# Anttwo/SuGaR

Hardware: NVIDIA B200
Metric: forward+backward views/sec @3M Gaussians 1920x1080 (higher is better)
Workload: dtype f32

## Files before the change

### sugar_b200/csrc/sgr_backward.cu

```cuda
#include <mutex>

#include "sgr_internal.cuh"

namespace sgr {

#ifndef SGR_BWD_PIPE3
#define SGR_BWD_PIPE3 1
#endif
#ifndef SGR_BWD_NS
#define SGR_BWD_NS 3
#endif
#ifndef SGR_BWD_B
#define SGR_BWD_B (SGR_BWD_PIPE3 ? 96 : 128)
#endif
constexpr int BWD_B = SGR_BWD_B;
constexpr int BWD_NW = 8;

__device__ __forceinline__ void red_add_v4(float *addr, float a, float b, float c, float d)
{
    asm volatile("red.global.add.v4.f32 [%0], {%1, %2, %3, %4};" ::"l"(addr), "f"(a), "f"(b), "f"(c), "f"(d) : "memory");
}
__device__ __forceinline__ void red_add_v2(float *addr, float a, float b)
{
    asm volatile("red.global.add.v2.f32 [%0], {%1, %2};" ::"l"(addr), "f"(a), "f"(b) : "memory");
// ... 304 lines not shown
                        dL_dalpha = fmaf(Cc.x - acc1, dp.y, dL_dalpha);
                        dL_dalpha = fmaf(Cc.y - acc2, dp.z, dL_dalpha);
                        dL_dalpha *= T;
                        dL_dalpha = fmaf(dp.w, inv, dL_dalpha);
                        S = B.z * dL_dalpha * G;
                        acc0 = fmaf(alpha, B.w, om * acc0);
                        acc1 = fmaf(alpha, Cc.x, om * acc1);
                        acc2 = fmaf(alpha, Cc.y, om * acc2);
                    }
                }
                sts64(cb + (lane * CH_PITCH + nfill) * 8, S, dchannel);
                const uint32_t ma = cb + CB_META + nfill * 32;
                sts128(ma, A.x, A.y, A.z, A.w);
                {
                    const float2 Cm = lds64(sc + j * 16 + 8);
                    sts128(ma + 16, B.x, B.z, Cm.x, Cm.y);
                }
                if (++nfill == CH) {
                    chunk_flush(cb, CH, blk_x0, blk_y0, 0.5f * W, 0.5f * H, gacc, dcol);
                    nfill = 0;
                }
            }
        }
#if SGR_BWD_PIPE3
        __syncwarp();
        if (lane == 0) mbar_arrive(&bars[NS + buf]);
#endif
    }
    if (nfill) chunk_flush(cb, nfill, blk_x0, blk_y0, 0.5f * W, 0.5f * H, gacc, dcol);
}

struct PreBwdArgs {
    int p0, p1;
    const float *means, *scales, *rots, *shs, *cov_pre;
    ViewConsts v;
    const int32_t *radii;
    const float *gacc;
    const float *dcol;
    float *dmeans2D, *dopacity, *dmeans3D, *dcov3D, *dsh, *dscales, *drots;
    float *rec11;
    int in_bulk_ok, out_bulk_ok, sh_stride, sh_vec;
    const float *sh_rest;
    const float4 *rec;
    float *dsh_rest;
    const float *const *view_tab;
    int nviews, my_view;
    size_t campos_off;
    float dsh_scale;
    float *const *stage_tab;
    int pf_off;
};

#define SH_C0 0.28209479177387814f
#define SH_C1 0.4886025119029199f
__constant__ float b_SH_C2[5] = {1.0925484305920792f, -1.0925484305920792f, 0.31539156525252005f,
                                 -1.0925484305920792f, 0.5462742152960396f};
__constant__ float b_SH_C3[7] = {-0.5900435899266435f, 2.890611442640554f, -0.4570457994644658f,
                                 0.3731763325901154f, -0.4570457994644658f, 1.445305721320277f,
                                 -0.5900435899266435f};

struct f3 {
    float x, y, z;
};

template <bool OTHERS = false>
__device__ __forceinline__ void sh_backward_inplace(int deg, int M, float *dc, float *rest, f3 dir_orig, f3 dRGB,
                                                    f3 &dmean, float out_scale = 1.0f, const float *oacc = nullptr)
{
    const f3 dS = {dRGB.x * out_scale, dRGB.y * out_scale, dRGB.z * out_scale};
    const float len = sqrtf(dir_orig.x * dir_orig.x + dir_orig.y * dir_orig.y + dir_orig.z * dir_orig.z);
    const float x = dir_orig.x / len, y = dir_orig.y / len, z = dir_orig.z / len;
    float ddx = 0.f, ddy = 0.f, ddz = 0.f;
#define SHB(k, w, cx, cy, cz)                                                          \
    {                                                                                  \
        float *q_ = (k) == 0 ? dc : rest + ((k) - 1) * 3;                              \
        const float t_ = q_[0] * dRGB.x + q_[1] * dRGB.y + q_[2] * dRGB.z;             \
        ddx += (cx) * t_;                                                              \
        ddy += (cy) * t_;                                                              \
        ddz += (cz) * t_;                                                              \
        const float w_ = (w);                                                          \
        if (OTHERS) {  \
            q_[0] = fmaf(w_, dS.x, oacc[(k) * 3]);                                     \
            q_[1] = fmaf(w_, dS.y, oacc[(k) * 3 + 1]);                                 \
            q_[2] = fmaf(w_, dS.z, oacc[(k) * 3 + 2]);                                 \
        } else {                                                                       \
            q_[0] = w_ * dS.x;                                                         \
            q_[1] = w_ * dS.y;                                                         \
            q_[2] = w_ * dS.z;                                                         \
        }                                                                              \
    }
    SHB(0, SH_C0, 0.f, 0.f, 0.f);
    if (deg > 0) {
        SHB(1, -SH_C1 * y, 0.f, -SH_C1, 0.f);
        SHB(2, SH_C1 * z, 0.f, 0.f, SH_C1);
        SHB(3, -SH_C1 * x, -SH_C1, 0.f, 0.f);
        if (deg > 1) {
            const float xx = x * x, yy = y * y, zz = z * z, xy = x * y, yz = y * z, xz = x * z;
            SHB(4, b_SH_C2[0] * xy, b_SH_C2[0] * y, b_SH_C2[0] * x, 0.f);
            SHB(5, b_SH_C2[1] * yz, 0.f, b_SH_C2[1] * z, b_SH_C2[1] * y);
            SHB(6, b_SH_C2[2] * (2.f * zz - xx - yy), b_SH_C2[2] * 2.f * -x, b_SH_C2[2] * 2.f * -y, b_SH_C2[2] * 2.f * 2.f * z);
            SHB(7, b_SH_C2[3] * xz, b_SH_C2[3] * z, 0.f, b_SH_C2[3] * x);
            SHB(8, b_SH_C2[4] * (xx - yy), b_SH_C2[4] * 2.f * x, b_SH_C2[4] * 2.f * -y, 0.f);
            if (deg > 2) {
                SHB(9, b_SH_C3[0] * y * (3.f * xx - yy), b_SH_C3[0] * 3.f * 2.f * xy, b_SH_C3[0] * 3.f * (xx - yy), 0.f);
                SHB(10, b_SH_C3[1] * xy * z, b_SH_C3[1] * yz, b_SH_C3[1] * xz, b_SH_C3[1] * xy);
                SHB(11, b_SH_C3[2] * y * (4.f * zz - xx - yy), b_SH_C3[2] * -2.f * xy,
                    b_SH_C3[2] * (-3.f * yy + 4.f * zz - xx), b_SH_C3[2] * 4.f * 2.f * yz);
                SHB(12, b_SH_C3[3] * z * (2.f * zz - 3.f * xx - 3.f * yy), b_SH_C3[3] * -3.f * 2.f * xz,
                    b_SH_C3[3] * -3.f * 2.f * yz, b_SH_C3[3] * 3.f * (2.f * zz - xx - yy));
                SHB(13, b_SH_C3[4] * x * (4.f * zz - xx - yy), b_SH_C3[4] * (-3.f * xx + 4.f * zz - yy),
                    b_SH_C3[4] * -2.f * xy, b_SH_C3[4] * 4.f * 2.f * xz);
                SHB(14, b_SH_C3[5] * z * (xx - yy), b_SH_C3[5] * 2.f * xz, b_SH_C3[5] * -2.f * yz, b_SH_C3[5] * (xx - yy));
                SHB(15, b_SH_C3[6] * x * (xx - 3.f * yy), b_SH_C3[6] * 3.f * (xx - yy), b_SH_C3[6] * -3.f * 2.f * xy, 0.f);
            }
        }
    }
#undef SHB
    for (int k = (deg + 1) * (deg + 1) * 3 - 3; k < (M - 1) * 3; k++) rest[k] = 0.f;
    const f3 o = dir_orig;
    const float sum2 = o.x * o.x + o.y * o.y + o.z * o.z;
    const float invsum32 = 1.0f / sqrtf(sum2 * sum2 * sum2);
    dmean.x += ((+sum2 - o.x * o.x) * ddx - o.y * o.x * ddy - o.z * o.x * ddz) * invsum32;
    dmean.y += (-o.x * o.y * ddx + (sum2 - o.y * o.y) * ddy - o.z * o.y * ddz) * invsum32;
    dmean.z += (-o.x * o.z * ddx - o.y * o.z * ddy + (sum2 - o.z * o.z) * ddz) * invsum32;
}

__device__ __forceinline__ void sh_accumulate(int deg, float *acc, f3 dir_orig, f3 g)
{
    const float inv = 1.0f / sqrtf(dir_orig.x * dir_orig.x + dir_orig.y * dir_orig.y + dir_orig.z * dir_orig.z);
    const float x = dir_orig.x * inv, y = dir_orig.y * inv, z = dir_orig.z * inv;
#define SHA(k, w)                                           \
    {                                                       \
        const float w_ = (w);                               \
        acc[(k) * 3] = fmaf(w_, g.x, acc[(k) * 3]);         \
        acc[(k) * 3 + 1] = fmaf(w_, g.y, acc[(k) * 3 + 1]); \
        acc[(k) * 3 + 2] = fmaf(w_, g.z, acc[(k) * 3 + 2]); \
    }
    SHA(0, SH_C0);
    if (deg > 0) {
        SHA(1, -SH_C1 * y);
        SHA(2, SH_C1 * z);
        SHA(3, -SH_C1 * x);
        if (deg > 1) {
            const float xx = x * x, yy = y * y, zz = z * z, xy = x * y, yz = y * z, xz = x * z;
            SHA(4, b_SH_C2[0] * xy);
            SHA(5, b_SH_C2[1] * yz);
            SHA(6, b_SH_C2[2] * (2.f * zz - xx - yy));
            SHA(7, b_SH_C2[3] * xz);
            SHA(8, b_SH_C2[4] * (xx - yy));
            if (deg > 2) {
                SHA(9, b_SH_C3[0] * y * (3.f * xx - yy));
// ... 35 lines not shown
__device__ __forceinline__ void bulk_s2g(void *dst, const void *src_smem, uint32_t bytes)
{
    asm volatile("cp.async.bulk.global.shared::cta.bulk_group [%0], [%1], %2;" ::"l"(dst), "r"(smem_u32(src_smem)),
                 "r"(bytes)
                 : "memory");
}

__device__ __forceinline__ void pb_stage(float *dst, const float *__restrict__ src, int n)
{
    for (int i = threadIdx.x; i < n; i += PB_T) dst[i] = __ldg(src + i);
}
__device__ __forceinline__ void pb_flush(float *__restrict__ dst, const float *src, int n)
{
    for (int i = threadIdx.x; i < n; i += PB_T) dst[i] = src[i];
}

template <bool RAW, bool MULTI = false>
__global__ void __launch_bounds__(PB_T) preprocess_backward_kernel(const PreBwdArgs a)
{
    extern __shared__ __align__(16) float sm[];
    __shared__ __align__(8) uint64_t s_bar;
    const int tid = threadIdx.x;
    const int base = a.p0 + blockIdx.x * PB_T;
    const int n = min(PB_T, a.p1 - base);
    const int i = base + tid;
    const int M = a.v.M;
    const bool full = (n == PB_T);

    if (a.in_bulk_ok && full) {
        if (tid == 0) {
            mbar_init(&s_bar, 1);
            mbar_fence_init();
            uint32_t bytes = PB_T * 32 + PB_T * 12;
            if (a.shs) bytes += PB_T * 12;
            if (RAW && a.shs) bytes += PB_T * 12 + PB_T * (uint32_t)(a.v.M - 1) * 12;
            if (a.scales) bytes += PB_T * 12 + PB_T * 16;
            if (a.cov_pre) bytes += PB_T * 24;
            const int pulled = MULTI ? min(a.nviews - 1, PB_VB) : 0;
            bytes += (uint32_t)pulled * PB_T * 12;
            mbar_expect_tx(&s_bar, bytes);
            for (int u = 0; u < pulled; u++) {
                const int v = u + (u >= a.my_view ? 1 : 0);
                bulk_g2s(sm + a.pf_off + u * PB_T * 3, a.view_tab[v] + (size_t)base * 3, PB_T * 12, &s_bar);
            }
            if (RAW && a.shs) {
                bulk_g2s(sm + PB_SHDC, a.shs + (size_t)base * 3, PB_T * 12, &s_bar);
                if (a.v.M > 1)
                    bulk_g2s(sm + PB_SH, a.sh_rest + (size_t)base * (a.v.M - 1) * 3, PB_T * (uint32_t)(a.v.M - 1) * 12, &s_bar);
            }
            bulk_g2s(sm + PB_GACC, a.gacc + (size_t)base * 8, PB_T * 32, &s_bar);
            if (a.shs) bulk_g2s(sm + PB_DCOL, a.dcol + (size_t)base * 3, PB_T * 12, &s_bar);
            bulk_g2s(sm + PB_MEANS, a.means + (size_t)base * 3, PB_T * 12, &s_bar);
            if (a.scales) {
                bulk_g2s(sm + PB_SCALES, a.scales + (size_t)base * 3, PB_T * 12, &s_bar);
                bulk_g2s(sm + PB_ROTS, a.rots + (size_t)base * 4, PB_T * 16, &s_bar);
            }
            if (a.cov_pre) bulk_g2s(sm + PB_COV, a.cov_pre + (size_t)base * 6, PB_T * 24, &s_bar);
        }
    } else {
        pb_stage(sm + PB_GACC, a.gacc + (size_t)base * 8, n * 8);
        if (a.shs) pb_stage(sm + PB_DCOL, a.dcol + (size_t)base * 3, n * 3);
        pb_stage(sm + PB_MEANS, a.means + (size_t)base * 3, n * 3);
        if (a.scales) {
            pb_stage(sm + PB_SCALES, a.scales + (size_t)base * 3, n * 3);
            pb_stage(sm + PB_ROTS, a.rots + (size_t)base * 4, n * 4);
        }
        if (a.cov_pre) pb_stage(sm + PB_COV, a.cov_pre + (size_t)base * 6, n * 6);
        if (RAW && a.shs) {
            pb_stage(sm + PB_SHDC, a.shs + (size_t)base * 3, n * 3);
            pb_stage(sm + PB_SH, a.sh_rest + (size_t)base * (M - 1) * 3, n * (M - 1) * 3);
        }
        if (MULTI) {
            const int pulled = min(a.nviews - 1, PB_VB);
            for (int u = 0; u < pulled; u++) {
                const int v = u + (u >= a.my_view ? 1 : 0);
                pb_stage(sm + a.pf_off + u * PB_T * 3, a.view_tab[v] + (size_t)base * 3, n * 3);
            }
        }
    }
    float *s_sh = sm + PB_SH;
    const int row_f = RAW ? (M - 1) * 3 : M * 3;
    if (!RAW && a.shs) {
        const float *src = a.shs + (size_t)base * row_f;
        if (a.sh_vec) {
            const int row_v = row_f >> 2, total = n * row_v;
            int r = tid / row_v, c = tid - r * row_v;
            const int dr = PB_T / row_v, dc = PB_T - dr * row_v;
            for (int k = tid; k < total; k += PB_T) {
                cp_async16(s_sh + r * a.sh_stride + c * 4, src + (size_t)k * 4);
                r += dr;
                c += dc;
                if (c >= row_v) {
                    c -= row_v;
                    r++;
                }
            }
        } else {
            const int total = n * row_f;
            for (int k = tid; k < total; k += PB_T) {
                const int r = k / row_f, c = k - r * row_f;
                cp_async4(s_sh + r * a.sh_stride + c, src + k);
            }
        }
        cp_async_commit();
    }
    int radius = 0;
    if (tid < n) radius = a.radii[i];
    const int others = MULTI ? a.nviews - 1 : 0;
    __syncthreads();
    if (a.in_bulk_ok && full) mbar_wait(&s_bar, 0);
    if (!RAW && a.shs) {
        cp_async_wait<0>();
        __syncthreads();
    }

    float oacc[MULTI ? 48 : 1];
    auto sum_other_views = [&]() {
        if (!MULTI) return;
#pragma unroll
        for (int k = 0; k < (MULTI ? 48 : 1); k++) oacc[k] = 0.f;
        if (others <= 0) return;
        const float mx = sm[PB_MEANS + tid * 3], my = sm[PB_MEANS + tid * 3 + 1], mz = sm[PB_MEANS + tid * 3 + 2];
        for (int u0 = 0; u0 < others; u0 += PB_VB) {
            float pf[PB_VB][3];
#pragma unroll
            for (int u = 0; u < PB_VB; u++) {
                const int uu = u0 + u, v = uu + (uu >= a.my_view ? 1 : 0);
                const bool on = uu < others;
                if (u0 == 0) {
                    const float *g = sm + a.pf_off + u * PB_T * 3 + tid * 3;
                    pf[u][0] = on ? g[0] : 0.f;
                    pf[u][1] = on ? g[1] : 0.f;
                    pf[u][2] = on ? g[2] : 0.f;
                } else {
                    const float *g = a.view_tab[on ? v : a.my_view] + (size_t)i * 3;
                    pf[u][0] = on ? __ldcg(g) : 0.f;
                    pf[u][1] = on ? __ldcg(g + 1) : 0.f;
                    pf[u][2] = on ? __ldcg(g + 2) : 0.f;
                }
            }
#pragma unroll
            for (int u = 0; u < PB_VB; u++) {
                const f3 g = {pf[u][0] * a.dsh_scale, pf[u][1] * a.dsh_scale, pf[u][2] * a.dsh_scale};
                if (g.x == 0.f && g.y == 0.f && g.z == 0.f) continue;
                const int uu = u0 + u, v = uu + (uu >= a.my_view ? 1 : 0);
                const float *cp = a.view_tab[v] + a.campos_off;
                sh_accumulate(a.v.D, oacc, {mx - __ldg(cp), my - __ldg(cp + 1), mz - __ldg(cp + 2)}, g);
            }
        }
    };
    if (MULTI && tid < n) sum_other_views();
    if (tid < n) {
        const bool vis = radius > 0;
        const bool aos = a.rec11 != nullptr;
        float *o_m2d = sm + PB_O_M2D + tid * 3, *o_cov = sm + PB_O_COV + tid * 6;
        float *o_m3d = aos ? sm + PB_O_R11 + tid * 11 : sm + PB_O_M3D + tid * 3;
        float *o_opa = aos ? o_m3d + 3 : sm + PB_O_OPA + tid;
        float *o_scl = aos ? o_m3d + 4 : sm + PB_O_SCL + tid * 3;
        float *o_rot = aos ? o_m3d + 7 : sm + PB_O_ROT + tid * 4;
        float *row = s_sh + tid * (RAW ? row_f : a.sh_stride);
        if (!vis) {
            o_m2d[0] = o_m2d[1] = o_m2d[2] = 0.f;
            *o_opa = 0.f;
            o_m3d[0] = o_m3d[1] = o_m3d[2] = 0.f;
#pragma unroll
            for (int k = 0; k < 6; k++) o_cov[k] = 0.f;
            o_scl[0] = o_scl[1] = o_scl[2] = 0.f;
            o_rot[0] = o_rot[1] = o_rot[2] = o_rot[3] = 0.f;
            if (a.shs && a.dsh) {
                if (MULTI) {
#pragma unroll
                    for (int k = 0; k < 48; k++)
                        if (k < row_f) row[k] = oacc[k];
                    for (int k = 48; k < row_f; k++) row[k] = 0.f;
                } else {
                    for (int k = 0; k < row_f; k++) row[k] = 0.f;
                }
                if (RAW) sm[PB_SHDC + tid * 3] = sm[PB_SHDC + tid * 3 + 1] = sm[PB_SHDC + tid * 3 + 2] = 0.f;
            }
        } else {
            const float4 *gr = (const float4 *)(sm + PB_GACC) + tid * 2;
            const float4 g0 = gr[0], g1 = gr[1];
            const float dmx = g0.x, dmy = g0.y;
            const float dcx = g0.z, dcy = g0.w, dcz = g1.x;
            o_m2d[0] = dmx;
            o_m2d[1] = dmy;
            o_m2d[2] = 0.f;
            float act_o = 1.0f;
            if (RAW) {
                const float o = __ldg(&a.rec[(size_t)i * 3 + 1]).z;
                act_o = o * (1.0f - o);
            }
            *o_opa = g1.y * act_o;

            const float *vm = a.v.viewmatrix, *proj = a.v.projmatrix;
            const float mx = sm[PB_MEANS + tid * 3], my = sm[PB_MEANS + tid * 3 + 1], mz = sm[PB_MEANS + tid * 3 + 2];
            float c3[6];
            float4 q = make_float4(1, 0, 0, 0);
            float sc0 = 0, sc1 = 0, sc2 = 0, q_len = 1.0f;
            if (a.cov_pre) {
#pragma unroll
                for (int k = 0; k < 6; k++) c3[k] = sm[PB_COV + tid * 6 + k];
// ... 47 lines not shown
                dcov[5] = (T0[2] * T0[2] * dL_da + T0[2] * T1[2] * dL_db + T1[2] * T1[2] * dL_dc);
                dcov[1] = 2 * T0[0] * T0[1] * dL_da + (T0[0] * T1[1] + T0[1] * T1[0]) * dL_db + 2 * T1[0] * T1[1] * dL_dc;
                dcov[2] = 2 * T0[0] * T0[2] * dL_da + (T0[0] * T1[2] + T0[2] * T1[0]) * dL_db + 2 * T1[0] * T1[2] * dL_dc;
                dcov[4] = 2 * T0[2] * T0[1] * dL_da + (T0[1] * T1[2] + T0[2] * T1[1]) * dL_db + 2 * T1[1] * T1[2] * dL_dc;
            } else {
#pragma unroll
                for (int k = 0; k < 6; k++) dcov[k] = 0.f;
            }
#pragma unroll
            for (int k = 0; k < 6; k++) o_cov[k] = dcov[k];
            float dT0[3], dT1[3];
#pragma unroll
            for (int k = 0; k < 3; k++) {
                dT0[k] = 2 * p[k] * dL_da + qv[k] * dL_db;
                dT1[k] = 2 * qv[k] * dL_dc + p[k] * dL_db;
            }
            const float dJ00 = vm[0] * dT0[0] + vm[4] * dT0[1] + vm[8] * dT0[2];
            const float dJ02 = vm[2] * dT0[0] + vm[6] * dT0[1] + vm[10] * dT0[2];
            const float dJ11 = vm[1] * dT1[0] + vm[5] * dT1[1] + vm[9] * dT1[2];
            const float dJ12 = vm[2] * dT1[0] + vm[6] * dT1[1] + vm[10] * dT1[2];
            const float tz = 1.f / tzv, tz2 = tz * tz, tz3 = tz2 * tz;
            const float dtx = x_grad_mul * -h_x * tz2 * dJ02;
            const float dty = y_grad_mul * -h_y * tz2 * dJ12;
            const float dtz = -h_x * tz2 * dJ00 - h_y * tz2 * dJ11 + (2 * h_x * tx) * tz3 * dJ02 + (2 * h_y * ty) * tz3 * dJ12;
            f3 dmean = {vm[0] * dtx + vm[1] * dty + vm[2] * dtz, vm[4] * dtx + vm[5] * dty + vm[6] * dtz,
                        vm[8] * dtx + vm[9] * dty + vm[10] * dtz};
            const float hw = xf_row(proj, 3, mx, my, mz);
            const float m_w = 1.0f / (hw + 0.0000001f);
            const float mul1 = (proj[0] * mx + proj[4] * my + proj[8] * mz + proj[12]) * m_w * m_w;
            const float mul2 = (proj[1] * mx + proj[5] * my + proj[9] * mz + proj[13]) * m_w * m_w;
            dmean.x += (proj[0] * m_w - proj[3] * mul1) * dmx + (proj[1] * m_w - proj[3] * mul2) * dmy;
            dmean.y += (proj[4] * m_w - proj[7] * mul1) * dmx + (proj[5] * m_w - proj[7] * mul2) * dmy;
            dmean.z += (proj[8] * m_w - proj[11] * mul1) * dmx + (proj[9] * m_w - proj[11] * mul2) * dmy;
            if (a.shs) {
                const f3 dRGB = {sm[PB_DCOL + tid * 3], sm[PB_DCOL + tid * 3 + 1], sm[PB_DCOL + tid * 3 + 2]};
                const float *cp = a.v.campos;
                sh_backward_inplace<MULTI>(a.v.D, M, RAW ? sm + PB_SHDC + tid * 3 : row, RAW ? row : row + 3,
                                           {mx - cp[0], my - cp[1], mz - cp[2]}, dRGB, dmean,
                                           MULTI ? a.dsh_scale : 1.0f, oacc);
            }
            o_m3d[0] = dmean.x;
            o_m3d[1] = dmean.y;
            o_m3d[2] = dmean.z;
            if (a.scales) {
                const float r = q.x, x = q.y, y = q.z, z = q.w;
                const float R[3][3] = {{1.f - 2.f * (y * y + z * z), 2.f * (x * y - r * z), 2.f * (x * z + r * y)},
                                       {2.f * (x * y + r * z), 1.f - 2.f * (x * x + z * z), 2.f * (y * z - r * x)},
                                       {2.f * (x * z - r * y), 2.f * (y * z + r * x), 1.f - 2.f * (x * x + y * y)}};
                const float s[3] = {a.v.scale_modifier * sc0, a.v.scale_modifier * sc1, a.v.scale_modifier * sc2};
                const float dS[3][3] = {{dcov[0], 0.5f * dcov[1], 0.5f * dcov[2]},
                                        {0.5f * dcov[1], dcov[3], 0.5f * dcov[4]},
                                        {0.5f * dcov[2], 0.5f * dcov[4], dcov[5]}};
                float dMt[3][3];
#pragma unroll
                for (int c = 0; c < 3; c++)
#pragma unroll
                    for (int w = 0; w < 3; w++)
                        dMt[w][c] = 2.0f * s[w] * R[0][w] * dS[c][0] + 2.0f * s[w] * R[1][w] * dS[c][1] +
                                    2.0f * s[w] * R[2][w] * dS[c][2];
#pragma unroll
                for (int k = 0; k < 3; k++) o_scl[k] = R[0][k] * dMt[k][0] + R[1][k] * dMt[k][1] + R[2][k] * dMt[k][2];
#pragma unroll
                for (int k = 0; k < 3; k++)
#pragma unroll
                    for (int w = 0; w < 3; w++) dMt[k][w] *= s[k];
                float4 dq;
                dq.x = 2 * z * (dMt[0][1] - dMt[1][0]) + 2 * y * (dMt[2][0] - dMt[0][2]) + 2 * x * (dMt[1][2] - dMt[2][1]);
                dq.y = 2 * y * (dMt[1][0] + dMt[0][1]) + 2 * z * (dMt[2][0] + dMt[0][2]) + 2 * r * (dMt[1][2] - dMt[2][1]) -
                       4 * x * (dMt[2][2] + dMt[1][1]);
                dq.z = 2 * x * (dMt[1][0] + dMt[0][1]) + 2 * r * (dMt[2][0] - dMt[0][2]) + 2 * z * (dMt[1][2] + dMt[2][1]) -
                       4 * y * (dMt[2][2] + dMt[0][0]);
                dq.w = 2 * r * (dMt[0][1] - dMt[1][0]) + 2 * x * (dMt[2][0] + dMt[0][2]) + 2 * y * (dMt[1][2] + dMt[2][1]) -
// ... 30 lines not shown
            } else {
                bulk_s2g(a.dopacity + base, sm + PB_O_OPA, PB_T * 4);
                bulk_s2g(a.dmeans3D + (size_t)base * 3, sm + PB_O_M3D, PB_T * 12);
                bulk_s2g(a.dscales + (size_t)base * 3, sm + PB_O_SCL, PB_T * 12);
                bulk_s2g(a.drots + (size_t)base * 4, sm + PB_O_ROT, PB_T * 16);
            }
            asm volatile("cp.async.bulk.commit_group;" ::: "memory");
        }
    } else {
        pb_flush(a.dmeans2D + (size_t)base * 3, sm + PB_O_M2D, n * 3);
        pb_flush(a.dcov3D + (size_t)base * 6, sm + PB_O_COV, n * 6);
        if (a.rec11) {
            pb_flush(rec_out + (size_t)base * 11, sm + PB_O_R11, n * 11);
        } else {
            pb_flush(a.dopacity + base, sm + PB_O_OPA, n);
            pb_flush(a.dmeans3D + (size_t)base * 3, sm + PB_O_M3D, n * 3);
            pb_flush(a.dscales + (size_t)base * 3, sm + PB_O_SCL, n * 3);
            pb_flush(a.drots + (size_t)base * 4, sm + PB_O_ROT, n * 4);
        }
    }
    if (RAW && a.dsh && M > 0) {
        if (out_bulk) {
            if (tid == 0) {
                bulk_s2g(a.dsh + (size_t)base * 3, sm + PB_SHDC, PB_T * 12);
                if (M > 1) bulk_s2g(a.dsh_rest + (size_t)base * row_f, sm + PB_SH, PB_T * (uint32_t)row_f * 4);
                asm volatile("cp.async.bulk.commit_group;" ::: "memory");
            }
        } else {
            pb_flush(a.dsh + (size_t)base * 3, sm + PB_SHDC, n * 3);
            pb_flush(a.dsh_rest + (size_t)base * row_f, sm + PB_SH, n * row_f);
        }
    } else if (a.dsh && M > 0) {
        float *dst = a.dsh + (size_t)base * row_f;
        if (a.shs) {
            if (a.sh_vec) {
                const int row_v = row_f >> 2, total = n * row_v;
                int r = tid / row_v, c = tid - r * row_v;
                const int dr = PB_T / row_v, dc = PB_T - dr * row_v;
                for (int k = tid; k < total; k += PB_T) {
                    ((float4 *)dst)[k] = *(const float4 *)(s_sh + r * a.sh_stride + c * 4);
                    r += dr;
                    c += dc;
                    if (c >= row_v) {
                        c -= row_v;
                        r++;
                    }
                }
            } else {
                const int total = n * row_f;
                for (int k = tid; k < total; k += PB_T) {
                    const int r = k / row_f, c = k - r * row_f;
                    dst[k] = s_sh[r * a.sh_stride + c];
                }
            }
        } else {
            for (int k = tid; k < n * row_f; k += PB_T) dst[k] = 0.f;
        }
    }
    if (out_bulk && tid == 0) asm volatile("cp.async.bulk.wait_group.read 0;" ::: "memory");
}

__device__ __forceinline__ const float *view_block(const float *base, size_t stride, const float *const *tab, int v)
{
    return tab ? tab[v] : base + (size_t)v * stride;
}

constexpr int SF_T = 256;
// ... 293 lines not shown
            static std::mutex mu;
            static cudaEvent_t evs[64][20] = {};
            int dev = 0;
            SGR_CUDA(cudaGetDevice(&dev));
            if (dev < 0 || dev >= 64 || ev_index < 0 || ev_index >= 20) {
                set_error("peer_signal_stream: device / chunk index out of range");
                return SGR_EINVAL;
            }
            std::lock_guard<std::mutex> lock(mu);
            if (!evs[dev][ev_index]) SGR_CUDA(cudaEventCreateWithFlags(&evs[dev][ev_index], cudaEventDisableTiming));
            sig = (cudaStream_t)plan->peer_signal_stream;
            SGR_CUDA(cudaEventRecord(evs[dev][ev_index], st));
            SGR_CUDA(cudaStreamWaitEvent(sig, evs[dev][ev_index], 0));
        }
        return sgr_peer_signal(plan->peer_flag_tab, plan->peer_nranks, slot, plan->peer_rank, plan->peer_seq, sig);
    };
    if (peer) {
        int rc = signal(plan->peer_slot_blend, 0, true);
        if (rc) return rc;
        if (plan->peer_view_blocks && dL_dsh && g->shs) {
            if (g->activations != 0 || !plan->peer_flags) {
                set_error("peer_view_blocks: needs peer_flags and activated (not raw) parameters");
                return SGR_EINVAL;
            }
            rc = sgr_peer_wait(plan->peer_flags, plan->peer_nranks, plan->peer_slot_blend, 1, plan->peer_seq,
                               plan->peer_timeout_s, st);
            if (rc) return rc;
        }
    }
    PreBwdArgs a;
    a.means = g->means3D;
    a.scales = g->scales;
    a.rots = g->rotations;
    a.shs = g->shs;
    a.cov_pre = g->cov3D_precomp;
    a.v.viewmatrix = view->viewmatrix;
    a.v.projmatrix = view->projmatrix;
    a.v.campos = view->campos;
    a.v.bg = view->bg;
    a.v.W = W;
    a.v.H = H;
    a.v.gx = gx;
    a.v.gy = gy;
    a.v.tanfovx = view->tanfovx;
    a.v.tanfovy = view->tanfovy;
    a.v.focal_y = H / (2.0f * view->tanfovy);
    a.v.focal_x = W / (2.0f * view->tanfovx);
    a.v.scale_modifier = view->scale_modifier;
    a.v.D = view->sh_degree;
    a.v.M = g->M;
    a.v.prefiltered = view->prefiltered;
    a.radii = radii;
    a.gacc = gacc;
    a.dcol = dL_dcolors;
    a.dmeans2D = dL_dmeans2D;
    a.dopacity = dL_dopacity;
    a.dmeans3D = dL_dmeans3D;
    a.dcov3D = dL_dcov3D;
    a.dsh = dL_dsh;
    a.dscales = dL_dscales;
    a.drots = dL_drotations;
    a.rec11 = rec11;
    a.view_tab = nullptr;
    a.stage_tab = nullptr;
    a.pf_off = 0;
    a.nviews = 1;
    a.my_view = 0;
    a.campos_off = (size_t)3 * P;
    a.dsh_scale = 1.0f;
    const bool raw = g->activations != 0;
    if (peer && plan->peer_view_blocks && dL_dsh && g->shs) {
        a.view_tab = (const float *const *)plan->peer_view_blocks;
        a.nviews = plan->peer_nranks;
        a.my_view = plan->peer_rank;
        a.dsh_scale = plan->peer_dsh_scale;
        a.stage_tab = (float *const *)plan->peer_record_stages;
        if (a.stage_tab && (!rec11 || PB_T != 64)) {
            set_error("peer_record_stages needs reduce_records (the local staging array) and 64-thread CTAs");
            return SGR_EINVAL;
        }
    }
    a.sh_rest = g->sh_rest;
    a.rec = geom.rec;
    a.dsh_rest = plan ? plan->dL_dsh_rest : nullptr;
    if (raw && g->shs && dL_dsh && g->M > 1 && !a.dsh_rest) {
        set_error("raw-parameter mode needs SgrBackwardPlan.dL_dsh_rest");
        return SGR_EINVAL;
    }
    auto al16 = [](const void *p) { return ((uintptr_t)p & 15u) == 0; };
    a.in_bulk_ok = al16(gacc) && al16(dL_dcolors) && al16(g->means3D) && (!g->scales || al16(g->scales)) &&
                   (!g->rotations || al16(g->rotations)) && (!g->cov3D_precomp || al16(g->cov3D_precomp)) &&
                   (!raw || !g->shs || (al16(g->shs) && (g->M == 1 || al16(g->sh_rest))));
    a.out_bulk_ok = al16(dL_dmeans2D) && al16(dL_dcov3D) &&
                    (rec11 ? al16(rec11) : (al16(dL_dopacity) && al16(dL_dmeans3D) && al16(dL_dscales) && al16(dL_drotations)));
    if (raw && g->shs && dL_dsh) a.out_bulk_ok = a.out_bulk_ok && al16(dL_dsh) && (g->M == 1 || al16(a.dsh_rest));
#ifdef SGR_PB_NO_BULK_STORE
    a.out_bulk_ok = 0;
#endif
    a.sh_stride = 0;
    a.sh_vec = 0;
    if (g->shs && !raw) {
        const int row_f = g->M * 3;
        if ((row_f % 4) == 0 && al16(g->shs) && al16(dL_dsh)) {
            int s4 = row_f / 4;
            if ((s4 & 1) == 0) s4 += 1;
            a.sh_stride = s4 * 4;
            a.sh_vec = 1;
        } else {
            a.sh_stride = (row_f & 1) ? row_f : row_f + 1;
        }
    }
    a.pf_off = PB_SH + PB_T * (raw ? (g->M > 0 ? (g->M - 1) * 3 : 0) : a.sh_stride);
    const int pulled = a.view_tab ? (a.nviews - 1 < PB_VB ? a.nviews - 1 : PB_VB) : 0;
    const size_t dyn = (size_t)(a.pf_off + pulled * PB_T * 3) * sizeof(float) + 16;
    int nchunks = plan && plan->num_chunks > 1 ? plan->num_chunks : 1;
    const int blocks = (P + PB_T - 1) / PB_T;
    if (nchunks > blocks) nchunks = blocks;
    int split_c = -1, split_p0 = 0, split_p1 = 0;
    auto side_event = [&](int index, cudaEvent_t *out) -> int {
        static std::mutex mu;
        static cudaEvent_t evs[64][20] = {};
        int dev = 0;
        SGR_CUDA(cudaGetDevice(&dev));
        if (dev < 0 || dev >= 64 || index < 0 || index >= 20) {
            set_error("peer_side_stream: device / chunk index out of range");
            return SGR_EINVAL;
        }
        std::lock_guard<std::mutex> lock(mu);
        if (!evs[dev][index]) SGR_CUDA(cudaEventCreateWithFlags(&evs[dev][index], cudaEventDisableTiming));
        *out = evs[dev][index];
        return SGR_OK;
    };
    auto split_chunk = [&](cudaStream_t B, int c, int p0, int p1) -> int {
        int rc = sgr_peer_wait(plan->peer_flags, plan->peer_nranks, plan->peer_slot_reduced0 + c, 1, plan->peer_seq,
                               plan->peer_timeout_s, B);
        if (rc) return rc;
        return finalize_impl(P, p0, p1, g->M, view->sh_degree, plan->peer_nranks, g->means3D, nullptr, nullptr, 0, 0, nullptr,
                             nullptr, plan->peer_sums, plan->peer_dsh_scale, dL_dmeans3D, dL_dopacity, dL_dscales,
                             dL_drotations, B, "peer exchange: bad arguments to the record split");
    };
    if (peer && plan->peer_side_stream &&
        (!plan->peer_rec_tab || !plan->peer_sum_tab || !plan->peer_sums || !plan->peer_flags || !rec11 || !dL_dmeans3D ||
         !dL_dopacity || !dL_dscales || !dL_drotations || nchunks > 16)) {
        set_error("peer_side_stream needs peer_rec_tab / peer_sum_tab / peer_sums / peer_flags, reduce_records, the four "
                  "record-bound gradient arrays and at most 16 chunks");
// ... 160 lines not shown
```

### sugar_b200/csrc/sgr_forward.cu

```cuda
#include <stdarg.h>
#include <stdio.h>

#include <mutex>
#include <vector>

#include "sgr_internal.cuh"

namespace sgr {

#ifndef SGR_PRE_T
#define SGR_PRE_T 128
#endif
constexpr int PRE_T = SGR_PRE_T;

struct PreArgs {
    int P;
    const float *means, *scales, *rots, *opac, *shs, *colors, *cov_pre;
    const float *sh_rest;
    ViewConsts v;
    int bulk_ok;
    int sh_stride;
    int sh_vec;
    GeomState geom;
    int32_t *radii;
// ... 13 lines not shown
#define SHK(k) ((k) == 0 ? dc[0] : rest[((k) - 1) * 3])
    float res = __fmul_rn(SH_C0, SHK(0));
    if (deg > 0) {
        res = __fmaf_rn(-__fmul_rn(y, SH_C1), SHK(1), res);
        res = __fmaf_rn(__fmul_rn(z, SH_C1), SHK(2), res);
        res = __fmaf_rn(-__fmul_rn(x, SH_C1), SHK(3), res);
        if (deg > 1) {
            const float xx = __fmul_rn(x, x), yy = __fmul_rn(y, y), zz = __fmul_rn(z, z);
            const float xy = __fmul_rn(x, y), yz = __fmul_rn(y, z), xz = __fmul_rn(x, z);
            const float zz2 = __fadd_rn(zz, zz);
            const float xx_yy = __fsub_rn(xx, yy);
            res = __fmaf_rn(__fmul_rn(xy, c_SH_C2[0]), SHK(4), res);
            res = __fmaf_rn(__fmul_rn(yz, c_SH_C2[1]), SHK(5), res);
            res = __fmaf_rn(__fmul_rn(__fsub_rn(__fsub_rn(zz2, xx), yy), c_SH_C2[2]), SHK(6), res);
            res = __fmaf_rn(__fmul_rn(xz, c_SH_C2[3]), SHK(7), res);
            res = __fmaf_rn(__fmul_rn(xx_yy, c_SH_C2[4]), SHK(8), res);
            if (deg > 2) {
                const float zz4_xx_yy = __fsub_rn(__fmaf_rn(zz, 4.0f, -xx), yy);
                res = __fmaf_rn(__fmul_rn(__fmul_rn(y, c_SH_C3[0]), __fmaf_rn(xx, 3.0f, -yy)), SHK(9), res);
                res = __fmaf_rn(__fmul_rn(__fmul_rn(xy, c_SH_C3[1]), z), SHK(10), res);
                res = __fmaf_rn(__fmul_rn(__fmul_rn(y, c_SH_C3[2]), zz4_xx_yy), SHK(11), res);
                res = __fmaf_rn(__fmul_rn(__fmul_rn(z, c_SH_C3[3]), __fmaf_rn(yy, -3.0f, __fmaf_rn(xx, -3.0f, zz2))),
                                SHK(12), res);
                res = __fmaf_rn(__fmul_rn(__fmul_rn(x, c_SH_C3[4]), zz4_xx_yy), SHK(13), res);
                res = __fmaf_rn(__fmul_rn(__fmul_rn(z, c_SH_C3[5]), xx_yy), SHK(14), res);
                res = __fmaf_rn(__fmul_rn(__fmul_rn(x, c_SH_C3[6]), __fmaf_rn(yy, -3.0f, xx)), SHK(15), res);
            }
        }
    }
#undef SHK
    return res;
}

__device__ __forceinline__ void stage_plain(float *dst, const float *__restrict__ src, int n)
{
    for (int i = threadIdx.x; i < n; i += PRE_T) dst[i] = __ldg(src + i);
}

template <bool RAW>
__global__ void __launch_bounds__(PRE_T) preprocess_kernel(const PreArgs a)
{
    extern __shared__ __align__(16) float s_sh[];
    __shared__ __align__(16) float s_means[PRE_T * 3];
    __shared__ __align__(16) float s_scales[PRE_T * 3];
    __shared__ __align__(16) float4 s_rots[PRE_T];
    __shared__ __align__(16) float s_opac[PRE_T];
    __shared__ __align__(16) float s_col[PRE_T * 3];
    __shared__ __align__(16) float s_cov[PRE_T * 6];
    __shared__ __align__(8) uint64_t s_bar;

    const int tid = threadIdx.x;
    const int base = blockIdx.x * PRE_T;
    const int n = min(PRE_T, a.P - base);
    const int idx = base + tid;
    const bool full = (n == PRE_T);

    if (a.bulk_ok && full) {
        if (tid == 0) {
            mbar_init(&s_bar, 1);
            mbar_fence_init();
            uint32_t bytes = PRE_T * 12 + PRE_T * 4;
            if (a.scales) bytes += PRE_T * 12 + PRE_T * 16;
            if (a.cov_pre) bytes += PRE_T * 24;
            if (a.colors) bytes += PRE_T * 12;
            if (RAW && a.shs) bytes += PRE_T * 12 + PRE_T * (uint32_t)(a.v.M - 1) * 12;
            mbar_expect_tx(&s_bar, bytes);
// ... 115 lines not shown
            s_live[tid] = visible ? 1 : 0;
            __syncthreads();
            stage_sh_rows(s_live);
        }
        cp_async_wait<0>();
        __syncthreads();
    }
    if (tid < n) {
        if (visible) {
            float r, g, b;
            uint32_t clamp_bits = 0;
            if (a.colors) {
                r = s_col[tid * 3], g = s_col[tid * 3 + 1], b = s_col[tid * 3 + 2];
            } else {
                const float *cp = a.v.campos;
                const float dx = __fsub_rn(mx, cp[0]), dy = __fsub_rn(my, cp[1]), dz = __fsub_rn(mz, cp[2]);
                const float len = __fsqrt_rn(__fmaf_rn(dz, dz, __fmaf_rn(dx, dx, __fmul_rn(dy, dy))));
                const float x = __fdiv_rn(dx, len), y = __fdiv_rn(dy, len), z = __fdiv_rn(dz, len);
                const float *dc, *rest;
                if (RAW) {
                    dc = s_col + tid * 3;
                    rest = s_sh + tid * (a.v.M - 1) * 3;
                } else {
                    dc = a.sh_stride ? s_sh + tid * a.sh_stride : a.shs + (size_t)idx * a.v.M * 3;
                    rest = dc + 3;
                }
                r = sh_channel(a.v.D, dc + 0, rest + 0, x, y, z);
                g = sh_channel(a.v.D, dc + 1, rest + 1, x, y, z);
                b = sh_channel(a.v.D, dc + 2, rest + 2, x, y, z);
                clamp_bits = (r < -0.5f ? 1u : 0u) | (g < -0.5f ? 2u : 0u) | (b < -0.5f ? 4u : 0u);
                r = (clamp_bits & 1u) ? 0.0f : __fadd_rn(r, 0.5f);
                g = (clamp_bits & 2u) ? 0.0f : __fadd_rn(g, 0.5f);
                b = (clamp_bits & 4u) ? 0.0f : __fadd_rn(b, 0.5f);
            }
            float tau;
            if (opacity * 255.0f > 1.0f) tau = -logf(opacity * 255.0f) - 1e-4f;
            else if (opacity == opacity) tau = __int_as_float(0x7f800000);
            else tau = -__int_as_float(0x7f800000);
            float4 *rec = a.geom.rec + (size_t)idx * 3;
            rec[0] = make_float4(px, py, con_a, con_b);
            rec[1] = make_float4(con_c, tau, opacity, r);
            rec[2] = make_float4(g, b, __uint_as_float(clamp_bits), __uint_as_float((uint32_t)idx));
            a.geom.depth[idx] = depth;
            a.geom.rect[idx] = make_ushort4((unsigned short)x0, (unsigned short)y0, (unsigned short)x1, (unsigned short)y1);
            a.radii[idx] = radius;
        } else {
            a.geom.rect[idx] = make_ushort4(0, 0, 0, 0);
            a.radii[idx] = 0;
        }
    }

    constexpr int SMALL = 6;
    const unsigned lane = tid & 31;
    const int rw = x1 - x0, rcnt = visible ? rw * (y1 - y0) : 0;
    if (rcnt > 0 && rcnt <= SMALL) {
        for (int ty = y0; ty < y1; ty++)
            for (int tx = x0; tx < x1; tx++) atomicAdd(a.tile_count + ty * a.v.gx + tx, 1u);
    }
    unsigned todo = __ballot_sync(0xffffffffu, rcnt > SMALL);
    while (todo) {
        const int src = __ffs(todo) - 1;
        todo &= todo - 1;
        const int rx0 = __shfl_sync(0xffffffffu, x0, src), ry0 = __shfl_sync(0xffffffffu, y0, src);
        const int w = __shfl_sync(0xffffffffu, rw, src), cnt = __shfl_sync(0xffffffffu, rcnt, src);
        for (int k = lane; k < cnt; k += 32) {
            const int ty = k / w, tx = k - ty * w;
// ... 899 lines not shown
```

### sugar_b200/csrc/sgr_internal.cuh

```cuda
#pragma once
#include <cuda_runtime.h>
#include <stdint.h>

#include "../../include/sugar_b200.h"

#define SGR_TILE 16
#define SGR_ALIGN 256

namespace sgr {

static inline size_t align_up(size_t v, size_t a = SGR_ALIGN) { return (v + a - 1) / a * a; }

struct GeomState {
    float4 *rec;
    ushort4 *rect;
    float *depth;
    static size_t bytes(size_t P) { return align_up(P * 48) + align_up(P * 8) + align_up(P * 4) + SGR_ALIGN; }
    static GeomState carve(void *base, size_t P)
    {
        char *p = (char *)align_up((size_t)base);
        GeomState s;
        s.rec = (float4 *)p; p += align_up(P * 48);
        s.rect = (ushort4 *)p; p += align_up(P * 8);
        s.depth = (float *)p;
        return s;
    }
};

struct ImageState {
    float *final_T;
    uint32_t *n_contrib;
    uint32_t *tile_count;
    uint32_t *tile_start;
    uint32_t *tile_cursor;
    uint32_t *tile_order;
    uint32_t *counters;
    static size_t bytes(size_t W, size_t H)
    {
        size_t T = ((W + 15) / 16) * ((H + 15) / 16);
        return 2 * align_up(W * H * 4) + 3 * align_up(T * 4) + align_up((T + 1) * 4) + align_up(64) + SGR_ALIGN;
    }
    static ImageState carve(void *base, size_t W, size_t H)
    {
        size_t T = ((W + 15) / 16) * ((H + 15) / 16);
        char *p = (char *)align_up((size_t)base);
        ImageState s;
        s.final_T = (float *)p; p += align_up(W * H * 4);
        s.n_contrib = (uint32_t *)p; p += align_up(W * H * 4);
        s.tile_count = (uint32_t *)p; p += align_up(T * 4);
        s.tile_start = (uint32_t *)p; p += align_up((T + 1) * 4);
        s.tile_cursor = (uint32_t *)p; p += align_up(T * 4);
        s.tile_order = (uint32_t *)p; p += align_up(T * 4);
        s.counters = (uint32_t *)p;
        return s;
    }
};

// ... 354 lines not shown
```

Baseline: 389.3.

## Precompute SH direction Jacobian in forward; stop loading SH coefficients in backward

```diff
diff --git a/sugar_b200/csrc/sgr_backward.cu b/sugar_b200/csrc/sgr_backward.cu
--- a/sugar_b200/csrc/sgr_backward.cu
+++ b/sugar_b200/csrc/sgr_backward.cu
@@ -360,15 +360,18 @@
 
 struct PreBwdArgs {
     int p0, p1;
-    const float *means, *scales, *rots, *shs, *cov_pre;
+    const float *means, *scales, *rots, *cov_pre;
+    int sh;
+    const float *ddir;
+    size_t ddir_stride;
     ViewConsts v;
     const int32_t *radii;
     const float *gacc;
     const float *dcol;
     float *dmeans2D, *dopacity, *dmeans3D, *dcov3D, *dsh, *dscales, *drots;
     float *rec11;
-    int in_bulk_ok, out_bulk_ok, sh_stride, sh_vec;
-    const float *sh_rest;
+    int in_bulk_ok, out_bulk_ok;
+    int sh_stride, sh_vec;
     const float4 *rec;
     float *dsh_rest;
     const float *const *view_tab;
@@ -392,20 +395,15 @@
 };
 
 template <bool OTHERS = false>
-__device__ __forceinline__ void sh_backward_inplace(int deg, int M, float *dc, float *rest, f3 dir_orig, f3 dRGB,
-                                                    f3 &dmean, float out_scale = 1.0f, const float *oacc = nullptr)
+__device__ __forceinline__ void sh_grad_row(int deg, int M, float *dc, float *rest, f3 dir_orig, f3 dRGB,
+                                            float out_scale = 1.0f, const float *oacc = nullptr)
 {
     const f3 dS = {dRGB.x * out_scale, dRGB.y * out_scale, dRGB.z * out_scale};
     const float len = sqrtf(dir_orig.x * dir_orig.x + dir_orig.y * dir_orig.y + dir_orig.z * dir_orig.z);
     const float x = dir_orig.x / len, y = dir_orig.y / len, z = dir_orig.z / len;
-    float ddx = 0.f, ddy = 0.f, ddz = 0.f;
-#define SHB(k, w, cx, cy, cz)                                                          \
+#define SHB(k, w)                                                                      \
     {                                                                                  \
         float *q_ = (k) == 0 ? dc : rest + ((k) - 1) * 3;                              \
-        const float t_ = q_[0] * dRGB.x + q_[1] * dRGB.y + q_[2] * dRGB.z;             \
-        ddx += (cx) * t_;                                                              \
-        ddy += (cy) * t_;                                                              \
-        ddz += (cz) * t_;                                                              \
         const float w_ = (w);                                                          \
         if (OTHERS) {  \
             q_[0] = fmaf(w_, dS.x, oacc[(k) * 3]);                                     \
@@ -417,34 +415,38 @@
             q_[2] = w_ * dS.z;                                                         \
         }                                                                              \
     }
-    SHB(0, SH_C0, 0.f, 0.f, 0.f);
+    SHB(0, SH_C0);
     if (deg > 0) {
-        SHB(1, -SH_C1 * y, 0.f, -SH_C1, 0.f);
-        SHB(2, SH_C1 * z, 0.f, 0.f, SH_C1);
-        SHB(3, -SH_C1 * x, -SH_C1, 0.f, 0.f);
+        SHB(1, -SH_C1 * y);
+        SHB(2, SH_C1 * z);
+        SHB(3, -SH_C1 * x);
         if (deg > 1) {
             const float xx = x * x, yy = y * y, zz = z * z, xy = x * y, yz = y * z, xz = x * z;
-            SHB(4, b_SH_C2[0] * xy, b_SH_C2[0] * y, b_SH_C2[0] * x, 0.f);
-            SHB(5, b_SH_C2[1] * yz, 0.f, b_SH_C2[1] * z, b_SH_C2[1] * y);
-            SHB(6, b_SH_C2[2] * (2.f * zz - xx - yy), b_SH_C2[2] * 2.f * -x, b_SH_C2[2] * 2.f * -y, b_SH_C2[2] * 2.f * 2.f * z);
-            SHB(7, b_SH_C2[3] * xz, b_SH_C2[3] * z, 0.f, b_SH_C2[3] * x);
-            SHB(8, b_SH_C2[4] * (xx - yy), b_SH_C2[4] * 2.f * x, b_SH_C2[4] * 2.f * -y, 0.f);
+            SHB(4, b_SH_C2[0] * xy);
+            SHB(5, b_SH_C2[1] * yz);
+            SHB(6, b_SH_C2[2] * (2.f * zz - xx - yy));
+            SHB(7, b_SH_C2[3] * xz);
+            SHB(8, b_SH_C2[4] * (xx - yy));
             if (deg > 2) {
-                SHB(9, b_SH_C3[0] * y * (3.f * xx - yy), b_SH_C3[0] * 3.f * 2.f * xy, b_SH_C3[0] * 3.f * (xx - yy), 0.f);
-                SHB(10, b_SH_C3[1] * xy * z, b_SH_C3[1] * yz, b_SH_C3[1] * xz, b_SH_C3[1] * xy);
-                SHB(11, b_SH_C3[2] * y * (4.f * zz - xx - yy), b_SH_C3[2] * -2.f * xy,
-                    b_SH_C3[2] * (-3.f * yy + 4.f * zz - xx), b_SH_C3[2] * 4.f * 2.f * yz);
-                SHB(12, b_SH_C3[3] * z * (2.f * zz - 3.f * xx - 3.f * yy), b_SH_C3[3] * -3.f * 2.f * xz,
-                    b_SH_C3[3] * -3.f * 2.f * yz, b_SH_C3[3] * 3.f * (2.f * zz - xx - yy));
-                SHB(13, b_SH_C3[4] * x * (4.f * zz - xx - yy), b_SH_C3[4] * (-3.f * xx + 4.f * zz - yy),
-                    b_SH_C3[4] * -2.f * xy, b_SH_C3[4] * 4.f * 2.f * xz);
-                SHB(14, b_SH_C3[5] * z * (xx - yy), b_SH_C3[5] * 2.f * xz, b_SH_C3[5] * -2.f * yz, b_SH_C3[5] * (xx - yy));
-                SHB(15, b_SH_C3[6] * x * (xx - 3.f * yy), b_SH_C3[6] * 3.f * (xx - yy), b_SH_C3[6] * -3.f * 2.f * xy, 0.f);
+                SHB(9, b_SH_C3[0] * y * (3.f * xx - yy));
+                SHB(10, b_SH_C3[1] * xy * z);
+                SHB(11, b_SH_C3[2] * y * (4.f * zz - xx - yy));
+                SHB(12, b_SH_C3[3] * z * (2.f * zz - 3.f * xx - 3.f * yy));
+                SHB(13, b_SH_C3[4] * x * (4.f * zz - xx - yy));
+                SHB(14, b_SH_C3[5] * z * (xx - yy));
+                SHB(15, b_SH_C3[6] * x * (xx - 3.f * yy));
             }
         }
     }
 #undef SHB
     for (int k = (deg + 1) * (deg + 1) * 3 - 3; k < (M - 1) * 3; k++) rest[k] = 0.f;
+}
+
+__device__ __forceinline__ void sh_dir_backward(const float *J, f3 dir_orig, f3 dRGB, f3 &dmean)
+{
+    const float ddx = J[0] * dRGB.x + J[3] * dRGB.y + J[6] * dRGB.z;
+    const float ddy = J[1] * dRGB.x + J[4] * dRGB.y + J[7] * dRGB.z;
+    const float ddz = J[2] * dRGB.x + J[5] * dRGB.y + J[8] * dRGB.z;
     const f3 o = dir_orig;
     const float sum2 = o.x * o.x + o.y * o.y + o.z * o.z;
     const float invsum32 = 1.0f / sqrtf(sum2 * sum2 * sum2);
@@ -546,8 +548,7 @@
             mbar_init(&s_bar, 1);
             mbar_fence_init();
             uint32_t bytes = PB_T * 32 + PB_T * 12;
-            if (a.shs) bytes += PB_T * 12;
-            if (RAW && a.shs) bytes += PB_T * 12 + PB_T * (uint32_t)(a.v.M - 1) * 12;
+            if (a.sh) bytes += PB_T * 12;
             if (a.scales) bytes += PB_T * 12 + PB_T * 16;
             if (a.cov_pre) bytes += PB_T * 24;
             const int pulled = MULTI ? min(a.nviews - 1, PB_VB) : 0;
@@ -557,13 +558,8 @@
                 const int v = u + (u >= a.my_view ? 1 : 0);
                 bulk_g2s(sm + a.pf_off + u * PB_T * 3, a.view_tab[v] + (size_t)base * 3, PB_T * 12, &s_bar);
             }
-            if (RAW && a.shs) {
-                bulk_g2s(sm + PB_SHDC, a.shs + (size_t)base * 3, PB_T * 12, &s_bar);
-                if (a.v.M > 1)
-                    bulk_g2s(sm + PB_SH, a.sh_rest + (size_t)base * (a.v.M - 1) * 3, PB_T * (uint32_t)(a.v.M - 1) * 12, &s_bar);
-            }
             bulk_g2s(sm + PB_GACC, a.gacc + (size_t)base * 8, PB_T * 32, &s_bar);
-            if (a.shs) bulk_g2s(sm + PB_DCOL, a.dcol + (size_t)base * 3, PB_T * 12, &s_bar);
+            if (a.sh) bulk_g2s(sm + PB_DCOL, a.dcol + (size_t)base * 3, PB_T * 12, &s_bar);
             bulk_g2s(sm + PB_MEANS, a.means + (size_t)base * 3, PB_T * 12, &s_bar);
             if (a.scales) {
                 bulk_g2s(sm + PB_SCALES, a.scales + (size_t)base * 3, PB_T * 12, &s_bar);
@@ -573,17 +569,13 @@
         }
     } else {
         pb_stage(sm + PB_GACC, a.gacc + (size_t)base * 8, n * 8);
-        if (a.shs) pb_stage(sm + PB_DCOL, a.dcol + (size_t)base * 3, n * 3);
+        if (a.sh) pb_stage(sm + PB_DCOL, a.dcol + (size_t)base * 3, n * 3);
         pb_stage(sm + PB_MEANS, a.means + (size_t)base * 3, n * 3);
         if (a.scales) {
             pb_stage(sm + PB_SCALES, a.scales + (size_t)base * 3, n * 3);
             pb_stage(sm + PB_ROTS, a.rots + (size_t)base * 4, n * 4);
         }
         if (a.cov_pre) pb_stage(sm + PB_COV, a.cov_pre + (size_t)base * 6, n * 6);
-        if (RAW && a.shs) {
-            pb_stage(sm + PB_SHDC, a.shs + (size_t)base * 3, n * 3);
-            pb_stage(sm + PB_SH, a.sh_rest + (size_t)base * (M - 1) * 3, n * (M - 1) * 3);
-        }
         if (MULTI) {
             const int pulled = min(a.nviews - 1, PB_VB);
             for (int u = 0; u < pulled; u++) {
@@ -594,39 +586,16 @@
     }
     float *s_sh = sm + PB_SH;
     const int row_f = RAW ? (M - 1) * 3 : M * 3;
-    if (!RAW && a.shs) {
-        const float *src = a.shs + (size_t)base * row_f;
-        if (a.sh_vec) {
-            const int row_v = row_f >> 2, total = n * row_v;
-            int r = tid / row_v, c = tid - r * row_v;
-            const int dr = PB_T / row_v, dc = PB_T - dr * row_v;
-            for (int k = tid; k < total; k += PB_T) {
-                cp_async16(s_sh + r * a.sh_stride + c * 4, src + (size_t)k * 4);
-                r += dr;
-                c += dc;
-                if (c >= row_v) {
-                    c -= row_v;
-                    r++;
-                }
-            }
-        } else {
-            const int total = n * row_f;
-            for (int k = tid; k < total; k += PB_T) {
-                const int r = k / row_f, c = k - r * row_f;
-                cp_async4(s_sh + r * a.sh_stride + c, src + k);
-            }
-        }
-        cp_async_commit();
-    }
     int radius = 0;
     if (tid < n) radius = a.radii[i];
+    float J[9];
+    if (a.sh && radius > 0) {
+#pragma unroll
+        for (int k = 0; k < 9; k++) J[k] = __ldg(a.ddir + k * a.ddir_stride + i);
+    }
     const int others = MULTI ? a.nviews - 1 : 0;
     __syncthreads();
     if (a.in_bulk_ok && full) mbar_wait(&s_bar, 0);
-    if (!RAW && a.shs) {
-        cp_async_wait<0>();
-        __syncthreads();
-    }
 
     float oacc[MULTI ? 48 : 1];
     auto sum_other_views = [&]() {
@@ -681,7 +650,7 @@
             for (int k = 0; k < 6; k++) o_cov[k] = 0.f;
             o_scl[0] = o_scl[1] = o_scl[2] = 0.f;
             o_rot[0] = o_rot[1] = o_rot[2] = o_rot[3] = 0.f;
-            if (a.shs && a.dsh) {
+            if (a.sh && a.dsh) {
                 if (MULTI) {
 #pragma unroll
                     for (int k = 0; k < 48; k++)
@@ -795,12 +764,14 @@
             dmean.x += (proj[0] * m_w - proj[3] * mul1) * dmx + (proj[1] * m_w - proj[3] * mul2) * dmy;
             dmean.y += (proj[4] * m_w - proj[7] * mul1) * dmx + (proj[5] * m_w - proj[7] * mul2) * dmy;
             dmean.z += (proj[8] * m_w - proj[11] * mul1) * dmx + (proj[9] * m_w - proj[11] * mul2) * dmy;
-            if (a.shs) {
+            if (a.sh) {
                 const f3 dRGB = {sm[PB_DCOL + tid * 3], sm[PB_DCOL + tid * 3 + 1], sm[PB_DCOL + tid * 3 + 2]};
                 const float *cp = a.v.campos;
-                sh_backward_inplace<MULTI>(a.v.D, M, RAW ? sm + PB_SHDC + tid * 3 : row, RAW ? row : row + 3,
-                                           {mx - cp[0], my - cp[1], mz - cp[2]}, dRGB, dmean,
-                                           MULTI ? a.dsh_scale : 1.0f, oacc);
+                const f3 dir = {mx - cp[0], my - cp[1], mz - cp[2]};
+                sh_dir_backward(J, dir, dRGB, dmean);
+                if (a.dsh)
+                    sh_grad_row<MULTI>(a.v.D, M, RAW ? sm + PB_SHDC + tid * 3 : row, RAW ? row : row + 3, dir, dRGB,
+                                       MULTI ? a.dsh_scale : 1.0f, oacc);
             }
             o_m3d[0] = dmean.x;
             o_m3d[1] = dmean.y;
@@ -897,7 +868,7 @@
         }
     } else if (a.dsh && M > 0) {
         float *dst = a.dsh + (size_t)base * row_f;
-        if (a.shs) {
+        if (a.sh) {
             if (a.sh_vec) {
                 const int row_v = row_f >> 2, total = n * row_v;
                 int r = tid / row_v, c = tid - r * row_v;
@@ -1257,7 +1228,9 @@
     a.means = g->means3D;
     a.scales = g->scales;
     a.rots = g->rotations;
-    a.shs = g->shs;
+    a.sh = g->shs != nullptr;
+    a.ddir = geom.ddir;
+    a.ddir_stride = geom.ddir_stride;
     a.cov_pre = g->cov3D_precomp;
     a.v.viewmatrix = view->viewmatrix;
     a.v.projmatrix = view->projmatrix;
@@ -1305,7 +1278,6 @@
             return SGR_EINVAL;
         }
     }
-    a.sh_rest = g->sh_rest;
     a.rec = geom.rec;
     a.dsh_rest = plan ? plan->dL_dsh_rest : nullptr;
     if (raw && g->shs && dL_dsh && g->M > 1 && !a.dsh_rest) {
@@ -1314,8 +1286,7 @@
     }
     auto al16 = [](const void *p) { return ((uintptr_t)p & 15u) == 0; };
     a.in_bulk_ok = al16(gacc) && al16(dL_dcolors) && al16(g->means3D) && (!g->scales || al16(g->scales)) &&
-                   (!g->rotations || al16(g->rotations)) && (!g->cov3D_precomp || al16(g->cov3D_precomp)) &&
-                   (!raw || !g->shs || (al16(g->shs) && (g->M == 1 || al16(g->sh_rest))));
+                   (!g->rotations || al16(g->rotations)) && (!g->cov3D_precomp || al16(g->cov3D_precomp));
     a.out_bulk_ok = al16(dL_dmeans2D) && al16(dL_dcov3D) &&
                     (rec11 ? al16(rec11) : (al16(dL_dopacity) && al16(dL_dmeans3D) && al16(dL_dscales) && al16(dL_drotations)));
     if (raw && g->shs && dL_dsh) a.out_bulk_ok = a.out_bulk_ok && al16(dL_dsh) && (g->M == 1 || al16(a.dsh_rest));
@@ -1324,9 +1295,9 @@
 #endif
     a.sh_stride = 0;
     a.sh_vec = 0;
-    if (g->shs && !raw) {
+    if (g->shs && dL_dsh && !raw) {
         const int row_f = g->M * 3;
-        if ((row_f % 4) == 0 && al16(g->shs) && al16(dL_dsh)) {
+        if ((row_f % 4) == 0 && al16(dL_dsh)) {
             int s4 = row_f / 4;
             if ((s4 & 1) == 0) s4 += 1;
             a.sh_stride = s4 * 4;
@@ -1335,7 +1306,8 @@
             a.sh_stride = (row_f & 1) ? row_f : row_f + 1;
         }
     }
-    a.pf_off = PB_SH + PB_T * (raw ? (g->M > 0 ? (g->M - 1) * 3 : 0) : a.sh_stride);
+    const int sh_rows = g->shs && dL_dsh ? (raw ? (g->M > 0 ? (g->M - 1) * 3 : 0) : a.sh_stride) : 0;
+    a.pf_off = PB_SH + PB_T * sh_rows;
     const int pulled = a.view_tab ? (a.nviews - 1 < PB_VB ? a.nviews - 1 : PB_VB) : 0;
     const size_t dyn = (size_t)(a.pf_off + pulled * PB_T * 3) * sizeof(float) + 16;
     int nchunks = plan && plan->num_chunks > 1 ? plan->num_chunks : 1;
diff --git a/sugar_b200/csrc/sgr_forward.cu b/sugar_b200/csrc/sgr_forward.cu
--- a/sugar_b200/csrc/sgr_forward.cu
+++ b/sugar_b200/csrc/sgr_forward.cu
@@ -69,6 +69,59 @@
     return res;
 }
 
+__device__ __forceinline__ void sh_dir_jacobian(int deg, const float *rest, float x, float y, float z, float *J)
+{
+#pragma unroll
+    for (int k = 0; k < 9; k++) J[k] = 0.f;
+    if (deg == 0) return;
+#define SHJ(k, d, w)                                                                      \
+    {                                                                                     \
+        const float w_ = (w);                                                             \
+        J[(d)] += rest[((k) - 1) * 3] * w_;                                               \
+        J[3 + (d)] += rest[((k) - 1) * 3 + 1] * w_;                                       \
+        J[6 + (d)] += rest[((k) - 1) * 3 + 2] * w_;                                       \
+    }
+    SHJ(1, 1, -SH_C1);
+    SHJ(2, 2, SH_C1);
+    SHJ(3, 0, -SH_C1);
+    if (deg > 1) {
+        const float xx = x * x, yy = y * y, zz = z * z, xy = x * y, yz = y * z, xz = x * z;
+        SHJ(4, 0, c_SH_C2[0] * y);
+        SHJ(4, 1, c_SH_C2[0] * x);
+        SHJ(5, 1, c_SH_C2[1] * z);
+        SHJ(5, 2, c_SH_C2[1] * y);
+        SHJ(6, 0, c_SH_C2[2] * -2.f * x);
+        SHJ(6, 1, c_SH_C2[2] * -2.f * y);
+        SHJ(6, 2, c_SH_C2[2] * 4.f * z);
+        SHJ(7, 0, c_SH_C2[3] * z);
+        SHJ(7, 2, c_SH_C2[3] * x);
+        SHJ(8, 0, c_SH_C2[4] * 2.f * x);
+        SHJ(8, 1, c_SH_C2[4] * -2.f * y);
+        if (deg > 2) {
+            SHJ(9, 0, c_SH_C3[0] * 6.f * xy);
+            SHJ(9, 1, c_SH_C3[0] * 3.f * (xx - yy));
+            SHJ(10, 0, c_SH_C3[1] * yz);
+            SHJ(10, 1, c_SH_C3[1] * xz);
+            SHJ(10, 2, c_SH_C3[1] * xy);
+            SHJ(11, 0, c_SH_C3[2] * -2.f * xy);
+            SHJ(11, 1, c_SH_C3[2] * (4.f * zz - xx - 3.f * yy));
+            SHJ(11, 2, c_SH_C3[2] * 8.f * yz);
+            SHJ(12, 0, c_SH_C3[3] * -6.f * xz);
+            SHJ(12, 1, c_SH_C3[3] * -6.f * yz);
+            SHJ(12, 2, c_SH_C3[3] * 3.f * (2.f * zz - xx - yy));
+            SHJ(13, 0, c_SH_C3[4] * (4.f * zz - 3.f * xx - yy));
+            SHJ(13, 1, c_SH_C3[4] * -2.f * xy);
+            SHJ(13, 2, c_SH_C3[4] * 8.f * xz);
+            SHJ(14, 0, c_SH_C3[5] * 2.f * xz);
+            SHJ(14, 1, c_SH_C3[5] * -2.f * yz);
+            SHJ(14, 2, c_SH_C3[5] * (xx - yy));
+            SHJ(15, 0, c_SH_C3[6] * 3.f * (xx - yy));
+            SHJ(15, 1, c_SH_C3[6] * -6.f * xy);
+        }
+    }
+#undef SHJ
+}
+
 __device__ __forceinline__ void stage_plain(float *dst, const float *__restrict__ src, int n)
 {
     for (int i = threadIdx.x; i < n; i += PRE_T) dst[i] = __ldg(src + i);
@@ -250,6 +303,10 @@
                 r = (clamp_bits & 1u) ? 0.0f : __fadd_rn(r, 0.5f);
                 g = (clamp_bits & 2u) ? 0.0f : __fadd_rn(g, 0.5f);
                 b = (clamp_bits & 4u) ? 0.0f : __fadd_rn(b, 0.5f);
+                float J[9];
+                sh_dir_jacobian(a.v.D, rest, x, y, z, J);
+#pragma unroll
+                for (int k = 0; k < 9; k++) a.geom.ddir[k * a.geom.ddir_stride + idx] = J[k];
             }
             float tau;
             if (opacity * 255.0f > 1.0f) tau = -logf(opacity * 255.0f) - 1e-4f;
diff --git a/sugar_b200/csrc/sgr_internal.cuh b/sugar_b200/csrc/sgr_internal.cuh
--- a/sugar_b200/csrc/sgr_internal.cuh
+++ b/sugar_b200/csrc/sgr_internal.cuh
@@ -15,14 +15,21 @@
     float4 *rec;
     ushort4 *rect;
     float *depth;
-    static size_t bytes(size_t P) { return align_up(P * 48) + align_up(P * 8) + align_up(P * 4) + SGR_ALIGN; }
+    float *ddir;
+    size_t ddir_stride;
+    static size_t bytes(size_t P)
+    {
+        return align_up(P * 48) + align_up(P * 8) + align_up(P * 4) + 9 * align_up(P * 4) + SGR_ALIGN;
+    }
     static GeomState carve(void *base, size_t P)
     {
         char *p = (char *)align_up((size_t)base);
         GeomState s;
         s.rec = (float4 *)p; p += align_up(P * 48);
         s.rect = (ushort4 *)p; p += align_up(P * 8);
-        s.depth = (float *)p;
+        s.depth = (float *)p; p += align_up(P * 4);
+        s.ddir = (float *)p;
+        s.ddir_stride = align_up(P * 4) / 4;
         return s;
     }
 };
```

Result: faster. 395.7, median of 6 (+1.6%).
